# SandeepaInduwaraSamaranayake/SwinVox

Hardware: AMD Instinct MI355X
Metric: views/sec fwd+bwd SwinVox-T 224^2, 32^3 voxel, n_views=8 (higher is better)
Workload: dtype bf16; 1 GPU; SwinVox-T full pipeline (ResNet50[:layer3] || Swin multi-stage, cross-view attention, decoder, merger, refiner), fwd+2xBCE+bwd, train mode, B=64 samples x V=8 views of 224x224 per GPU; global_batch=64, n_views=8, images_per_gpu=512, parallelism=single GPU, launch=eager (one host launch per kernel, three streams)

## Files before the change

swinvox_amd/csrc/stencil.hip:

```cpp
#include "common.h"
#include <map>
#include <mutex>
#include <type_traits>

namespace sv {

constexpr int TZ = 4, TY = 8, TX = 8;
constexpr int HZ = TZ + 2, HY = TY + 2, HX = TX + 2;
constexpr int HPOS = HZ * HY * HX;
constexpr int NVOX = TZ * TY * TX;
typedef __attribute__((address_space(3))) bf16x4 lds_bf16x4_t;

__device__ __forceinline__ bf16x4 to_bf16x4(float4 v) {
  bf16x4 b;
  b[0] = (__bf16)v.x; b[1] = (__bf16)v.y; b[2] = (__bf16)v.z; b[3] = (__bf16)v.w;
  return b;
}
__device__ __forceinline__ bf16x4 to_bf16x4(bf16x4 v) { return v; }

__device__ __forceinline__ int xcd_first_tile() {
  const int n = gridDim.x, b = blockIdx.x;
  return (n & 7) == 0 ? (b & 7) * (n >> 3) + (b >> 3) : b;
}

struct TileId { int img, z0, y0, x0; };
template <int TZV = TZ>
__device__ __forceinline__ TileId tile_of(int t, int D, int H, int W) {
  const int tz = D / TZV, ty = H / TY, tx = W / TX;
  TileId r;
  r.x0 = (t % tx) * TX; t /= tx; r.y0 = (t % ty) * TY; t /= ty; r.z0 = (t % tz) * TZV; r.img = t / tz;
  return r;
}

template <int G, typename AT, int TZV = TZ, int NTHR = 256>
struct HaloRegs {
  static constexpr int HZV = TZV + 2, HPOSV = HZV * HY * HX;
  static constexpr int C = 16 * G, VPP = C / 4, N = (HPOSV * VPP + NTHR - 1) / NTHR;
  typedef typename std::conditional<G == 1, int, long long>::type OffT;
  typename V4<AT>::type r[N];
  OffT off[N];
  int face[N];
  int lds[N];
  __device__ __forceinline__ void init(int ldx, long long plane, int cin_load, int H, int W, int tid, int pitch = HX) {
#pragma unroll
    for (int k = 0; k < N; ++k) {
      const int i = tid + NTHR * k;
      const int h = i / VPP, v = i - h * VPP;
      const int hx = h % HX; const int t2 = h / HX; const int hy = t2 % HY; const int hz = t2 / HY;
      const int cv = v * 4, pl = plane ? cv / ldx : 0;
      face[k] = (hz == 0 ? 1 : 0) | (hz == HZV - 1 ? 2 : 0) | (hy == 0 ? 4 : 0) | (hy == HY - 1 ? 8 : 0) | (hx == 0 ? 16 : 0) | (hx == HX - 1 ? 32 : 0) |
                ((i < HPOSV * VPP && cv < cin_load) ? 0 : 64);
      off[k] = (OffT)pl * (OffT)plane + (OffT)(((hz * H + hy) * W + hx) * ldx + (cv - pl * ldx));
      lds[k] = ((hz * HY + hy) * pitch + hx) * C + cv;
    }
  }
  __device__ __forceinline__ void load(const AT* __restrict__ x, int ldx, const TileId& t, int D, int H, int W) {
    const int out = (t.z0 == 0 ? 1 : 0) | (t.z0 + TZV == D ? 2 : 0) | (t.y0 == 0 ? 4 : 0) | (t.y0 + TY == H ? 8 : 0) | (t.x0 == 0 ? 16 : 0) | (t.x0 + TX == W ? 32 : 0) | 64;
    const AT* corner = x + ((((long long)t.img * D + t.z0 - 1) * H + t.y0 - 1) * W + t.x0 - 1) * (long long)ldx;
#pragma unroll
    for (int k = 0; k < N; ++k) {
      typename V4<AT>::type q = V4<AT>::zero();
#ifndef SV_ST_PROBE_NOLOAD
      if ((face[k] & out) == 0) q = V4<AT>::load(corner + off[k]);
#endif
      r[k] = q;
    }
  }
  __device__ __forceinline__ void store(__bf16* Xs, int tid) const {
#pragma unroll
    for (int k = 0; k < N; ++k) {
      const int i = tid + NTHR * k;
      if (i < HPOSV * VPP) *reinterpret_cast<bf16x4*>(Xs + lds[k]) = to_bf16x4(r[k]);
    }
  }
};

template <typename AT>
struct StencilArgsT {
  const AT* x; int ldx; int cin_load;
  long long x_plane, out_plane;
  const __bf16* w;
  const float* bias; AT* out; int ldc; int col_off; int cout;
  const AT* residual; int ldr;
  double* stats;
  int I, D, H, W, ntiles;
};

template <int G> struct StencilPitch { static constexpr int HXP = G == 1 ? 16 : HX; };
template <int G> struct StencilBrick { static constexpr int TZV = 8, NTHR = TZV * 64; };
template <int G> struct StencilBrickF { static constexpr int TZV = 8, NTHR = TZV * 64; };
template <int G, int NT, typename AT, bool VEC>
__global__ __launch_bounds__(StencilBrickF<G>::NTHR, 2) void stencil3_fwd_kernel(const StencilArgsT<AT> p) {
  constexpr int C = 16 * G, KTOT = 27 * C, KPAD = (KTOT + 31) / 32 * 32, NSTEP = KPAD / 32, HXP = StencilPitch<G>::HXP;
  constexpr int TZV = StencilBrickF<G>::TZV, NTHR = StencilBrickF<G>::NTHR, NW = NTHR / 64;
  __shared__ __attribute__((aligned(16))) char xc[(TZV + 2) * HY * HXP * C * 2];
  __shared__ __attribute__((aligned(16))) __bf16 Ws[NT * 16 * KPAD];
  __shared__ float red[16 * 16 * 2];
  __bf16* Xs = reinterpret_cast<__bf16*>(xc);
  const int tid = threadIdx.x, lane = tid & 63, wave = tid >> 6;
  const int lr = lane & 15, lg = lane >> 4;

  for (int i = tid; i < NT * 16 * KPAD / 8; i += NTHR) {
    const int n = (i * 8) / KPAD, k = (i * 8) - n * KPAD;
    bf16x8 v = VecN<__bf16, 8>::zero();
    if (k < KTOT) v = *reinterpret_cast<const bf16x8*>(p.w + (size_t)n * KTOT + k);
    *reinterpret_cast<bf16x8*>(Ws + n * KPAD + k) = v;
  }
  const int cs4 = (p.cout + 3) & ~3;
  float bias4[NT][4], st1[4] = {0.f, 0.f, 0.f, 0.f}, st2[4] = {0.f, 0.f, 0.f, 0.f};
#pragma unroll
  for (int nt = 0; nt < NT; ++nt)
#pragma unroll
    for (int j = 0; j < 4; ++j) { const int n = nt * 16 + lg * 4 + j; bias4[nt][j] = (p.bias && n < p.cout) ? p.bias[n] : 0.f; }

  HaloRegs<G, AT, TZV, NTHR> hr;
  hr.init(p.ldx, p.x_plane, p.cin_load, p.H, p.W, tid, HXP);
  int tile = xcd_first_tile();
  TileId t = tile_of<TZV>(tile < p.ntiles ? tile : 0, p.D, p.H, p.W);
  if (tile < p.ntiles) { hr.load(p.x, p.ldx, t, p.D, p.H, p.W); hr.store(Xs, tid); }
  __syncthreads();
  const int yy = lr >> 3, xx = lr & 7;
  int toff[NSTEP];
#pragma unroll
  for (int s = 0; s < NSTEP; ++s) {
    const int kb = s * 32 + lg * 8;
    int tap = kb / C; const int c = kb - tap * C;
    if (tap > 26) tap = 26;
    const int dz = tap / 9, dy = (tap - dz * 9) / 3, dx = tap - dz * 9 - dy * 3;
    toff[s] = (((dz * HY + dy) * HXP + dx) * C + c) * 2;
  }
  const char* xrow = xc + ((wave * HY + yy) * HXP + xx) * C * 2;
  const char* wrow = reinterpret_cast<const char*>(Ws) + (lr * KPAD + lg * 8) * 2;
  const int n0 = lg * 4;
  bool colreal[NT][4];
#pragma unroll
  for (int nt = 0; nt < NT; ++nt)
#pragma unroll
    for (int j = 0; j < 4; ++j) colreal[nt][j] = nt * 16 + n0 + j < p.cout;
  for (; tile < p.ntiles; tile += gridDim.x) {
    const int next = tile + gridDim.x;
    TileId tn = t;
    if (next < p.ntiles) { tn = tile_of<TZV>(next, p.D, p.H, p.W); hr.load(p.x, p.ldx, tn, p.D, p.H, p.W); }

    f32x4 acc[4][NT];
#pragma unroll
    for (int mt = 0; mt < 4; ++mt)
#pragma unroll
      for (int nt = 0; nt < NT; ++nt) acc[mt][nt] = (f32x4){0.f, 0.f, 0.f, 0.f};
#ifndef SV_ST_PROBE_NOMMA
#pragma unroll
    for (int s = 0; s < NSTEP; ++s) {
      bf16x8 b[NT];
#pragma unroll
      for (int nt = 0; nt < NT; ++nt) b[nt] = *reinterpret_cast<const bf16x8*>(wrow + nt * 16 * KPAD * 2 + s * 64);
      const char* ap = xrow + toff[s];
#pragma unroll
      for (int mt = 0; mt < 4; ++mt) {
        const bf16x8 a = *reinterpret_cast<const bf16x8*>(ap + mt * (2 * HXP * C * 2));
#pragma unroll
        for (int nt = 0; nt < NT; ++nt) acc[mt][nt] = __builtin_amdgcn_mfma_f32_16x16x32_bf16(b[nt], a, acc[mt][nt], 0, 0, 0);
      }
    }
#endif
    const size_t pos0 = (((size_t)t.img * p.D + t.z0 + wave) * p.H + t.y0 + yy) * p.W + t.x0 + xx;
    if constexpr (VEC) {
#pragma unroll
      for (int nt = 0; nt < NT; ++nt) {
        const int nn = nt * 16 + n0;
        if (nn >= cs4) continue;
        AT* orow; const AT* rrow = nullptr;
        if (p.out_plane) { const int pl = nn / p.ldc; orow = p.out + (size_t)pl * p.out_plane + pos0 * p.ldc + (nn - pl * p.ldc); }
        else orow = p.out + pos0 * p.ldc + p.col_off + nn;
        if (p.residual) rrow = p.residual + pos0 * p.ldr + nn;
#pragma unroll
        for (int mt = 0; mt < 4; ++mt) {
          float v[4];
#pragma unroll
          for (int j = 0; j < 4; ++j) v[j] = colreal[nt][j] ? acc[mt][nt][j] + bias4[nt][j] : 0.f;
          if (NT == 1 && p.stats) {
#pragma unroll
            for (int j = 0; j < 4; ++j) { st1[j] += v[j]; st2[j] += v[j] * v[j]; }
          }
          if (p.residual) {
            const float4 rv = ld4f(rrow + (size_t)mt * 2 * p.W * p.ldr);
            v[0] += rv.x; v[1] += rv.y; v[2] += rv.z; v[3] += rv.w;
          }
#ifdef SV_ST_PROBE_NOSTORE
          if (v[0] == 1234.5f)
#endif
          st4f(orow + (size_t)mt * 2 * p.W * p.ldc, make_float4(v[0], v[1], v[2], v[3]));
        }
      }
    } else {
#pragma unroll
      for (int mt = 0; mt < 4; ++mt) {
        const size_t pos = pos0 + (size_t)mt * 2 * p.W;
#pragma unroll
        for (int nt = 0; nt < NT; ++nt) {
          const int nn = nt * 16 + n0;
#pragma unroll
          for (int j = 0; j < 4; ++j) {
            if (nn + j < p.cout) {
              float r = acc[mt][nt][j] + bias4[nt][j];
              if (NT == 1 && p.stats) { st1[j] += r; st2[j] += r * r; }
              if (p.residual) r += ldf(p.residual + pos * p.ldr + nn + j);
              stf(p.out + pos * p.ldc + p.col_off + nn + j, r);
            }
          }
        }
      }
    }
    t = tn;
    __syncthreads();
    if (next < p.ntiles) hr.store(Xs, tid);
    __syncthreads();
  }
  if (NT == 1 && p.stats) {
#pragma unroll
    for (int j = 0; j < 4; ++j) {
      { st1[j] += dpp_move<0xB1>(st1[j]); st1[j] += dpp_move<0x4E>(st1[j]); st1[j] += dpp_move<0x141>(st1[j]); st1[j] += dpp_move<0x140>(st1[j]);
        st2[j] += dpp_move<0xB1>(st2[j]); st2[j] += dpp_move<0x4E>(st2[j]); st2[j] += dpp_move<0x141>(st2[j]); st2[j] += dpp_move<0x140>(st2[j]); }
    }
    if (lr == 0) {
#pragma unroll
      for (int j = 0; j < 4; ++j) { red[(wave * 16 + lg * 4 + j) * 2] = st1[j]; red[(wave * 16 + lg * 4 + j) * 2 + 1] = st2[j]; }
    }
    __syncthreads();
    if (tid < 16 && tid < p.cout) {
      float a = 0.f, b = 0.f;
#pragma unroll
      for (int w = 0; w < NW; ++w) { a += red[(w * 16 + tid) * 2]; b += red[(w * 16 + tid) * 2 + 1]; }
      double* st = p.stats + (size_t)(blockIdx.x % SV_BN_SLOTS) * 2 * p.cout;
      atomicAdd(st + tid, (double)a);
      atomicAdd(st + p.cout + tid, (double)b);
    }
  }
}

template <typename AT>
struct StencilWArgsT {
  const AT* x; int ldx; int cin_load;
  long long x_plane;
  const AT* dy; int lddy; int cout_load;
  float* dw;
  float* ws;
  float* dbias;
  int cout, cin;
  int c_stride, c_valid;
  int I, D, H, W, ntiles;
};

constexpr int WG_SLOTS = 16;
__global__ __launch_bounds__(256) void stencil_wgrad_fold_kernel(const float* __restrict__ ws, float* __restrict__ dw, int n) {
  const int i = blockIdx.x * 256 + threadIdx.x;
  if (i >= n) return;
  float a = 0.f;
#pragma unroll
  for (int sl = 0; sl < WG_SLOTS; ++sl) a += ws[(size_t)sl * n + i];
  dw[i] += a;
}

template <int G, typename AT>
__global__ __launch_bounds__(StencilBrick<G>::NTHR, 2) void stencil3_wgrad_kernel(const StencilWArgsT<AT> p) {
  constexpr int C = 16 * G, TZV = StencilBrick<G>::TZV, NTHR = StencilBrick<G>::NTHR, NW = NTHR / 64, NTAPW = (27 + NW - 1) / NW;
  constexpr int HPOSV = (TZV + 2) * HY * HX, NVOXV = TZV * TY * TX;
  __shared__ __attribute__((aligned(16))) __bf16 Xs[HPOSV * C];
  __shared__ __attribute__((aligned(16))) __bf16 Ds[NVOXV * 16];
  __shared__ float bred[NTHR / 16 * 16];
  const int tid = threadIdx.x, lane = tid & 63, wave = tid >> 6;
  const int lr = lane & 15, lg = lane >> 4, q = lr >> 2, pp = lr & 3;
  const int ntap = (27 - wave + NW - 1) / NW;
  f32x4 acc[NTAPW][G];
#pragma unroll
  for (int i = 0; i < NTAPW; ++i)
#pragma unroll
    for (int gg = 0; gg < G; ++gg) acc[i][gg] = (f32x4){0.f, 0.f, 0.f, 0.f};
  float bsum = 0.f;

  HaloRegs<G, AT, TZV, NTHR> hr;
  hr.init(p.ldx, p.x_plane, p.cin_load, p.H, p.W, tid);
  typename V4<AT>::type dr[4];
  auto load_dy = [&](const TileId& t) {
#pragma unroll
    for (int k = 0; k < 4; ++k) {
      const int i = tid + NTHR * k;
      const int v = i >> 2, c4 = i & 3;
      const int xx = v % TX; const int t2 = v / TX; const int yy = t2 % TY; const int zz = t2 / TY;
      typename V4<AT>::type qv = V4<AT>::zero();
      if (c4 * 4 < p.cout_load)
        qv = V4<AT>::load(p.dy + ((((size_t)t.img * p.D + t.z0 + zz) * p.H + t.y0 + yy) * p.W + t.x0 + xx) * (size_t)p.lddy + c4 * 4);
      dr[k] = qv;
    }
  };
  auto store_dy = [&]() {
#pragma unroll
    for (int k = 0; k < 4; ++k) *reinterpret_cast<bf16x4*>(Ds + (tid + NTHR * k) * 4) = to_bf16x4(dr[k]);
  };

  int tile = xcd_first_tile();
  if (tile < p.ntiles) {
    const TileId t = tile_of<TZV>(tile, p.D, p.H, p.W);
    hr.load(p.x, p.ldx, t, p.D, p.H, p.W); load_dy(t);
    hr.store(Xs, tid); store_dy();
  }
  __syncthreads();
  for (; tile < p.ntiles; tile += gridDim.x) {
    const int next = tile + gridDim.x;
    if (next < p.ntiles) {
      const TileId t = tile_of<TZV>(next, p.D, p.H, p.W);
      hr.load(p.x, p.ldx, t, p.D, p.H, p.W); load_dy(t);
    }
    if (p.dbias) {
      const int c = tid & 15, vg = tid >> 4;
#pragma unroll
      for (int k = 0; k < 16; ++k) bsum += (float)Ds[(vg * 16 + k) * 16 + c];
    }
#pragma unroll 1
    for (int ch = 0; ch < 2 * TZV; ++ch) {
      const int z = ch >> 1, yb = (ch & 1) * 4 + lg;
      const __bf16* asrc = Ds + (((z * TY + yb) * TX) + q) * 16 + pp * 4;
      const bf16x4 alo = __builtin_amdgcn_ds_read_tr16_b64_v4bf16((lds_bf16x4_t*)(asrc));
      const bf16x4 ahi = __builtin_amdgcn_ds_read_tr16_b64_v4bf16((lds_bf16x4_t*)(asrc + 4 * 16));
      const bf16x8 a = __builtin_shufflevector(alo, ahi, 0, 1, 2, 3, 4, 5, 6, 7);
#pragma unroll
      for (int i = 0; i < NTAPW; ++i) {
        if (i < ntap) {
          const int tap = wave + NW * i;
          const int dz = tap / 9, dy = (tap - dz * 9) / 3, dx = tap - dz * 9 - dy * 3;
          const int hb = ((z + dz) * HY + yb + dy) * HX + dx + q;
#pragma unroll
          for (int gg = 0; gg < G; ++gg) {
            const __bf16* bsrc = Xs + hb * C + gg * 16 + pp * 4;
            const bf16x4 blo = __builtin_amdgcn_ds_read_tr16_b64_v4bf16((lds_bf16x4_t*)(bsrc));
            const bf16x4 bhi = __builtin_amdgcn_ds_read_tr16_b64_v4bf16((lds_bf16x4_t*)(bsrc + 4 * C));
            const bf16x8 b = __builtin_shufflevector(blo, bhi, 0, 1, 2, 3, 4, 5, 6, 7);
            acc[i][gg] = __builtin_amdgcn_mfma_f32_16x16x32_bf16(a, b, acc[i][gg], 0, 0, 0);
          }
        }
      }
    }
    __syncthreads();
    if (next < p.ntiles) { hr.store(Xs, tid); store_dy(); }
    __syncthreads();
  }
  if (p.dbias) {
    bred[tid] = bsum;
    __syncthreads();
    if (tid < 16 && tid < p.cout) {
      float a = 0.f;
#pragma unroll
      for (int g2 = 0; g2 < NTHR / 16; ++g2) a += bred[g2 * 16 + tid];
      atomicAdd(p.dbias + tid, a);
    }
  }
  float* dst = p.ws ? p.ws + (size_t)(blockIdx.x % WG_SLOTS) * p.cout * p.cin * 27 : p.dw;
#pragma unroll
  for (int i = 0; i < NTAPW; ++i) {
    if (i < ntap) {
      const int tap = wave + NW * i;
#pragma unroll
      for (int gg = 0; gg < G; ++gg) {
        const int cm = gg * 16 + lr;
        const int grp = cm / p.c_stride, within = cm - grp * p.c_stride;
        const int ci = grp * p.c_valid + within;
        if (within < p.c_valid && ci < p.cin) {
#pragma unroll
          for (int j = 0; j < 4; ++j) {
            const int co = lg * 4 + j;
            if (co < p.cout) atomicAdd(dst + ((size_t)co * p.cin + ci) * 27 + tap, acc[i][gg][j]);
          }
        }
      }
    }
  }
}

struct TConv4Args {
  const __bf16* x; const __bf16* w;
  const float* bias; __bf16* out; double* stats; int cout; int I, D, H, W, nbricks;
};
constexpr int T4_JZ = 4, T4_JY = 4, T4_JX = 8, T4_HZ = 6, T4_HY = 6, T4_HX = 10, T4_HPOS = T4_HZ * T4_HY * T4_HX;

__global__ __launch_bounds__(256, 2) void tconv4s2_fwd_kernel(const TConv4Args p) {
  __shared__ __attribute__((aligned(16))) __bf16 Xs[T4_HPOS * 32];
  __shared__ __attribute__((aligned(16))) __bf16 Ws[8 * 8 * 256];
  __shared__ __attribute__((aligned(16))) __bf16 Os[8 * 8 * 16 * 8];
  __shared__ float red[4][16];
  const int tid = threadIdx.x, lane = tid & 63, wave = tid >> 6;
  const int lr = lane & 15, lg = lane >> 4;
  for (int i = tid; i < 8 * 8 * 256 / 8; i += 256) {
    const int c8 = (i & 3) * 8, t = (i >> 2) & 7, co = (i >> 5) & 7, cls = i >> 8;
    const int az = cls >> 2, ay = (cls >> 1) & 1, ax = cls & 1, dz = t >> 2, dy = (t >> 1) & 1, dx = t & 1;
    const int kz = az ? 2 - 2 * dz : 3 - 2 * dz, ky = ay ? 2 - 2 * dy : 3 - 2 * dy, kx = ax ? 2 - 2 * dx : 3 - 2 * dx;
    bf16x8 v = VecN<__bf16, 8>::zero();
    if (co < p.cout) v = *reinterpret_cast<const bf16x8*>(p.w + ((size_t)co * 64 + (kz * 4 + ky) * 4 + kx) * 32 + c8);
    *reinterpret_cast<bf16x8*>(Ws + ((cls * 8 + co) * 256) + t * 32 + c8) = v;
  }
  float bias4[4];
#pragma unroll
  for (int j = 0; j < 4; ++j) bias4[j] = (p.bias && lg < 2 && lg * 4 + j < p.cout) ? p.bias[lg * 4 + j] : 0.f;
  double st1[8], st2[8];
#pragma unroll
  for (int c = 0; c < 8; ++c) { st1[c] = 0.0; st2[c] = 0.0; }
  const int bz = p.D / T4_JZ, by = p.H / T4_JY, bx = p.W / T4_JX;
  __syncthreads();
  for (int brick = blockIdx.x; brick < p.nbricks; brick += gridDim.x) {
    int t = brick;
    const int x0 = (t % bx) * T4_JX; t /= bx;
    const int y0 = (t % by) * T4_JY; t /= by;
    const int z0 = (t % bz) * T4_JZ; const int img = t / bz;
    for (int i = tid; i < T4_HPOS * 4; i += 256) {
      const int h = i >> 2, c8 = (i & 3) * 8;
      const int hx = h % T4_HX; const int t2 = h / T4_HX; const int hy = t2 % T4_HY; const int hz = t2 / T4_HY;
      const int z = z0 - 1 + hz, y = y0 - 1 + hy, xx = x0 - 1 + hx;
      bf16x8 v = VecN<__bf16, 8>::zero();
      if ((unsigned)z < (unsigned)p.D && (unsigned)y < (unsigned)p.H && (unsigned)xx < (unsigned)p.W)
        v = *reinterpret_cast<const bf16x8*>(p.x + ((((size_t)img * p.D + z) * p.H + y) * p.W + xx) * 32 + c8);
      *reinterpret_cast<bf16x8*>(Xs + h * 32 + c8) = v;
    }
    __syncthreads();
    const int yy = lr >> 3, xx = lr & 7;
#pragma unroll 1
    for (int ci = 0; ci < 2; ++ci) {
      const int cls = 2 * wave + ci, az = cls >> 2, ay = (cls >> 1) & 1, ax = cls & 1;
      bf16x8 b[8];
#pragma unroll
      for (int tt = 0; tt < 8; ++tt) {
        b[tt] = VecN<__bf16, 8>::zero();
        if (lr < 8) b[tt] = *reinterpret_cast<const bf16x8*>(Ws + (cls * 8 + lr) * 256 + tt * 32 + lg * 8);
      }
#pragma unroll 2
      for (int g = 0; g < 8; ++g) {
        const int jz = g >> 1, jy = (g & 1) * 2 + yy;
        const int base = ((jz + az) * T4_HY + (jy + ay)) * T4_HX + (xx + ax);
        f32x4 acc = (f32x4){0.f, 0.f, 0.f, 0.f};
#pragma unroll
        for (int tt = 0; tt < 8; ++tt) {
          const int off = ((tt >> 2) * T4_HY + ((tt >> 1) & 1)) * T4_HX + (tt & 1);
          const bf16x8 a = *reinterpret_cast<const bf16x8*>(Xs + (base + off) * 32 + lg * 8);
          acc = __builtin_amdgcn_mfma_f32_16x16x32_bf16(b[tt], a, acc, 0, 0, 0);
        }
        if (lg < 2) {
          bf16x4 o;
#pragma unroll
          for (int j = 0; j < 4; ++j) o[j] = (__bf16)(acc[j] + bias4[j]);
          const int oz = 2 * jz + az, oy = 2 * jy + ay, ox = 2 * xx + ax;
          *reinterpret_cast<bf16x4*>(Os + ((oz * 8 + oy) * 16 + ox) * 8 + lg * 4) = o;
        }
      }
    }
    __syncthreads();
#pragma unroll
    for (int k = 0; k < 4; ++k) {
      const int v = tid + 256 * k;
      const int ox = v & 15, oy = (v >> 4) & 7, oz = v >> 7;
      const bf16x8 o = *reinterpret_cast<const bf16x8*>(Os + v * 8);
      const size_t pos = (((size_t)img * (2 * p.D) + 2 * z0 + oz) * (2 * p.H) + 2 * y0 + oy) * (2 * p.W) + 2 * x0 + ox;
      *reinterpret_cast<bf16x8*>(p.out + pos * 8) = o;
      if (p.stats) {
#pragma unroll
        for (int c = 0; c < 8; ++c) { const double f = (double)(float)o[c]; st1[c] += f; st2[c] += f * f; }
      }
    }
    __syncthreads();
  }
  if (p.stats) {
#pragma unroll
    for (int c = 0; c < 8; ++c) {
      float a = (float)st1[c], b2 = (float)st2[c];
      a = wave_sum(a); b2 = wave_sum(b2);
      if (lane == 0) { red[wave][c] = a; red[wave][8 + c] = b2; }
    }
    __syncthreads();
    if (tid < 16 && (tid & 7) < p.cout) {
      const float v = red[0][tid] + red[1][tid] + red[2][tid] + red[3][tid];
      double* st = p.stats + (size_t)(blockIdx.x % SV_BN_SLOTS) * 2 * p.cout;
      atomicAdd(st + (tid >> 3) * p.cout + (tid & 7), (double)v);
    }
  }
}

}

using namespace sv;

static int resident_per_cu(const void* kernel, int threads = 256) {
  static std::mutex mu;
  static std::map<const void*, int> cache;
  std::lock_guard<std::mutex> lk(mu);
  auto it = cache.find(kernel);
  if (it != cache.end()) return it->second;
  int n = 0;
  if (hipOccupancyMaxActiveBlocksPerMultiprocessor(&n, kernel, threads, 0) != hipSuccess || n < 1) { (void)hipGetLastError(); n = 1; }
  cache[kernel] = n;
  return n;
}

static int stencil_check(int I, int D, int H, int W) {
  SV_REQUIRE(I > 0 && D % 8 == 0 && H % TY == 0 && W % TX == 0, "stencil3: grid %dx%dx%d must be a multiple of the 8x8x8 brick", D, H, W);
  return SV_OK;
}

#define SV_STENCIL_LAUNCH(GG, NTT, VV)                                                                                     \
  do {                                                                                                                    \
    constexpr int nthr = StencilBrickF<GG>::NTHR;                                                                         \
    const int nt_ = I * (D / StencilBrickF<GG>::TZV) * (H / TY) * (W / TX);                                               \
    a.ntiles = nt_;                                                                                                       \
    const int resident = 256 * resident_per_cu((const void*)stencil3_fwd_kernel<GG, NTT, AT, VV>, nthr);                  \
    hipLaunchKernelGGL((stencil3_fwd_kernel<GG, NTT, AT, VV>), dim3(nt_ < resident ? nt_ : resident), dim3(nthr), 0, s, a); \
  } while (0)

extern "C" int sv_stencil3_fwd(const void* x, int ldx, int cin_load, int groups, const void* w_bf16, int ntiles16,
                               const float* bias, void* out, int ldc, int col_off, int cout, const void* residual, int ldr,
                               double* stats, int I, int D, int H, int W, long long x_plane_stride, long long out_plane_stride,
                               int act_dtype, void* stream) {
  SV_REQUIRE(x && w_bf16 && out, "stencil3_fwd: null argument");
  SV_REQUIRE(x_plane_stride >= 0 && out_plane_stride >= 0 && x_plane_stride % 4 == 0 && out_plane_stride % 4 == 0, "stencil3_fwd: bad plane strides");
  SV_REQUIRE(!out_plane_stride || (col_off == 0 && !residual && ldc % 4 == 0 && cout % ldc == 0),
             "stencil3_fwd: planar output needs col_off == 0, no residual and whole planes of ldc (multiple of 4) columns");
  SV_REQUIRE_ACT(act_dtype);
  if (int rc = stencil_check(I, D, H, W)) return rc;
    SV_REQUIRE(cin_load % 4 == 0 && cin_load <= 16 * groups && ldx % 4 == 0 && (x_plane_stride ? cin_load % ldx == 0 : ldx >= cin_load),
             "stencil3_fwd: bad input channels (cin_load=%d ldx=%d groups=%d)", cin_load, ldx, groups);
  SV_REQUIRE(cout > 0 && cout <= 16 * ntiles16 && (out_plane_stride || ldc >= col_off + cout), "stencil3_fwd: bad output window");
  SV_REQUIRE(!stats || ntiles16 == 1, "stencil3_fwd: statistics need a single 16-column tile");
  const uintptr_t amask = act_dtype == SV_BF16 ? 7 : 15;
  SV_REQUIRE(((uintptr_t)x & amask) == 0 && ((uintptr_t)w_bf16 & 15) == 0, "stencil3_fwd: operands must be aligned to 4 elements");
  SV_REQUIRE((ldc & 3) != 0 || (((uintptr_t)out | (uintptr_t)residual) & amask) == 0,
             "stencil3_fwd: out/residual must be aligned to 4 elements when ldc is a multiple of 4");
  const int ntiles = I * (D / TZ) * (H / TY) * (W / TX);
  hipStream_t s = (hipStream_t)stream;
  if (!((groups == 1 && ntiles16 == 1) || (groups == 3 && ntiles16 == 1) || (groups == 1 && ntiles16 == 3))) {
    set_error("stencil3_fwd: unsupported (groups=%d, ntiles16=%d)", groups, ntiles16);
    return SV_ERR_INVALID;
  }
  SV_DISPATCH_ACT(act_dtype,
    const int cs4 = (cout + 3) & ~3;
    const bool vec = out_plane_stride != 0 || ((ldc & 3) == 0 && (col_off & 3) == 0 && col_off + cs4 <= ldc && (!residual || ((ldr & 3) == 0 && cs4 <= ldr)));
    StencilArgsT<AT> a{static_cast<const AT*>(x), ldx, cin_load, x_plane_stride, out_plane_stride, (const __bf16*)w_bf16, bias, static_cast<AT*>(out), ldc, col_off, cout,
                       static_cast<const AT*>(residual), ldr, stats, I, D, H, W, ntiles};
    if (groups == 1 && ntiles16 == 1) { if (vec) SV_STENCIL_LAUNCH(1, 1, true); else SV_STENCIL_LAUNCH(1, 1, false); }
    else if (groups == 3) { if (vec) SV_STENCIL_LAUNCH(3, 1, true); else SV_STENCIL_LAUNCH(3, 1, false); }
    else { if (vec) SV_STENCIL_LAUNCH(1, 3, true); else SV_STENCIL_LAUNCH(1, 3, false); });
  return check_launch("sv_stencil3_fwd");
}

extern "C" size_t sv_stencil3_wgrad_workspace_floats(int cout, int cin) { return (size_t)WG_SLOTS * cout * cin * 27; }

extern "C" int sv_stencil3_wgrad(const void* x, int ldx, int cin_load, int groups, const void* dy, int lddy, int cout_load,
                                 float* dw, float* dbias, float* workspace, int cout, int cin, int c_stride, int c_valid, int I, int D, int H,
                                 int W, long long x_plane_stride, int act_dtype, void* stream) {
  SV_REQUIRE(x && dy && dw, "stencil3_wgrad: null argument");
  SV_REQUIRE(x_plane_stride >= 0 && x_plane_stride % 4 == 0 && (!x_plane_stride || cin_load % ldx == 0), "stencil3_wgrad: bad plane stride");
  SV_REQUIRE_ACT(act_dtype);
  if (int rc = stencil_check(I, D, H, W)) return rc;
  SV_REQUIRE(cin_load % 4 == 0 && cin_load <= 16 * groups && ldx % 4 == 0 && cout_load % 4 == 0 && cout_load <= 16 && lddy % 4 == 0,
             "stencil3_wgrad: bad channel layout");
  SV_REQUIRE(cout > 0 && cout <= 16 && cin > 0 && c_stride > 0 && c_valid > 0, "stencil3_wgrad: bad channel counts");
  SV_REQUIRE((((uintptr_t)x | (uintptr_t)dy) & (act_dtype == SV_BF16 ? 7 : 15)) == 0, "stencil3_wgrad: operands must be aligned to 4 elements");
  SV_REQUIRE(groups == 1 || groups == 3, "stencil3_wgrad: unsupported groups=%d", groups);
    const int ntiles = I * (D / (groups == 3 ? StencilBrick<3>::TZV : StencilBrick<1>::TZV)) * (H / TY) * (W / TX);
  hipStream_t s = (hipStream_t)stream;
  SV_DISPATCH_ACT(act_dtype,
    const int per_cu = groups == 1 ? resident_per_cu((const void*)stencil3_wgrad_kernel<1, AT>, StencilBrick<1>::NTHR)
                                   : resident_per_cu((const void*)stencil3_wgrad_kernel<3, AT>, StencilBrick<3>::NTHR);
    const int resident = 256 * per_cu;
    const int blocks = ntiles < resident ? ntiles : resident;
    StencilWArgsT<AT> a{static_cast<const AT*>(x), ldx, cin_load, x_plane_stride, static_cast<const AT*>(dy), lddy, cout_load, dw, workspace, dbias, cout, cin, c_stride, c_valid,
                        I, D, H, W, ntiles};
    if (groups == 1) hipLaunchKernelGGL((stencil3_wgrad_kernel<1, AT>), dim3(blocks), dim3(StencilBrick<1>::NTHR), 0, s, a);
    else hipLaunchKernelGGL((stencil3_wgrad_kernel<3, AT>), dim3(blocks), dim3(StencilBrick<3>::NTHR), 0, s, a););
  if (workspace) hipLaunchKernelGGL(stencil_wgrad_fold_kernel, dim3(cdiv(cout * cin * 27, 256)), dim3(256), 0, s, workspace, dw, cout * cin * 27);
  return check_launch("sv_stencil3_wgrad");
}

extern "C" int sv_tconv4s2_fwd(const void* x, const void* w_packed, const float* bias, void* out, double* stats, int I, int D, int H, int W,
                               int cin, int cout, void* stream) {
  SV_REQUIRE(x && w_packed && out && I > 0, "tconv4s2_fwd: null argument");
  SV_REQUIRE(cin == 32 && cout > 0 && cout <= 8, "tconv4s2_fwd: built for 32 input and <= 8 output channels (got %d -> %d)", cin, cout);
  SV_REQUIRE(D % T4_JZ == 0 && H % T4_JY == 0 && W % T4_JX == 0, "tconv4s2_fwd: input grid %dx%dx%d must be a multiple of the 4x4x8 brick", D, H, W);
  SV_REQUIRE((((uintptr_t)x | (uintptr_t)w_packed | (uintptr_t)out) & 15) == 0, "tconv4s2_fwd: operands must be 16-byte aligned");
  TConv4Args a{static_cast<const __bf16*>(x), static_cast<const __bf16*>(w_packed), bias, static_cast<__bf16*>(out), stats, cout, I, D, H, W,
               I * (D / T4_JZ) * (H / T4_JY) * (W / T4_JX)};
  const int blocks = a.nbricks < 512 ? a.nbricks : 512;
  hipLaunchKernelGGL(tconv4s2_fwd_kernel, dim3(blocks), dim3(256), 0, (hipStream_t)stream, a);
  return check_launch("sv_tconv4s2_fwd");
}
```

Baseline: 4896 views/s.

## Add z-sweep wgrad kernel for 3x3x3 stencil reusing dy slices across taps

Adds a new weight-gradient kernel for the 3D stencil conv, enabled by default with an env opt-out. Each wave owns a pair of in-plane taps and sweeps the z slices of a brick, reusing each loaded dy and x fragment across the three dz taps via MFMA with transposed LDS reads. The halo loader is restructured into z-slice groups so fewer per-thread offsets are held in registers. The two y-halves combine their accumulators through LDS before the atomics. The trade-offs are more accumulator registers, a different occupancy setting and added code complexity.

```diff
diff --git a/swinvox_amd/csrc/stencil.hip b/swinvox_amd/csrc/stencil.hip
--- a/swinvox_amd/csrc/stencil.hip
+++ b/swinvox_amd/csrc/stencil.hip
@@ -72,6 +72,67 @@
       const int i = tid + NTHR * k;
       if (i < HPOSV * VPP) *reinterpret_cast<bf16x4*>(Xs + lds[k]) = to_bf16x4(r[k]);
     }
+  }
+};
+
+template <int G, typename AT, int TZV, int NTHR>
+struct HaloSliceRegs {
+  static constexpr int HZV = TZV + 2, C = 16 * G, VPP = C / 4;
+  static constexpr int ZG = G == 1 ? 5 : 2, NGRP = HZV / ZG, GV = ZG * HY * HX * VPP, NP = (GV + NTHR - 1) / NTHR, N = NGRP * NP;
+  static_assert(HZV % ZG == 0, "groups of whole z-slices");
+  static_assert(HZV * HY * 16 * C < (1 << 20), "LDS offsets (pitch <= 16 positions) take 20 bits");
+  typename V4<AT>::type r[N];
+  int off[NP], meta[NP];
+  long long plane_;
+  int gstep_, lstep_;
+  __device__ __forceinline__ void init(int ldx, long long plane, int cin_load, int H, int W, int tid, int pitch) {
+#pragma unroll
+    for (int j = 0; j < NP; ++j) {
+      const int i = tid + NTHR * j;
+      int h = i / VPP, v = i - h * VPP;
+      const int nvp = ldx / 4;
+      if (plane && VPP % nvp == 0) {
+        const int row = i / (HX * VPP), rem = i - row * (HX * VPP);
+        const int pq = rem / (HX * nvp), r2 = rem - pq * (HX * nvp), px = r2 / nvp;
+        h = row * HX + px; v = pq * nvp + (r2 - px * nvp);
+      }
+      const int hx = h % HX; const int t2 = h / HX; const int hy = t2 % HY; const int hz = t2 / HY;
+      const int cv = v * 4, pl = plane ? cv / ldx : 0;
+      const int fc = (hz == 0 ? 1 : 0) | (hz == ZG - 1 ? 2 : 0) | (hy == 0 ? 4 : 0) | (hy == HY - 1 ? 8 : 0) | (hx == 0 ? 16 : 0) | (hx == HX - 1 ? 32 : 0) |
+                     ((i < GV && cv < cin_load) ? 0 : 64);
+      const int lo = i < GV ? ((hz * HY + hy) * pitch + hx) * C + cv : 0;
+      meta[j] = lo | (fc << 20) | (pl << 27);
+      off[j] = ((hz * H + hy) * W + hx) * ldx + (cv - pl * ldx);
+    }
+    plane_ = plane; gstep_ = ZG * H * W * ldx; lstep_ = ZG * HY * pitch * C;
+  }
+  __device__ __forceinline__ void load(const AT* __restrict__ x, int ldx, const TileId& t, int D, int H, int W) {
+    const int zlo = t.z0 == 0 ? 1 : 0, zhi = t.z0 + TZV == D ? 2 : 0;
+    const int yx = (t.y0 == 0 ? 4 : 0) | (t.y0 + TY == H ? 8 : 0) | (t.x0 == 0 ? 16 : 0) | (t.x0 + TX == W ? 32 : 0) | 64;
+    const AT* corner = x + ((((long long)t.img * D + t.z0 - 1) * H + t.y0 - 1) * W + t.x0 - 1) * (long long)ldx;
+#pragma unroll
+    for (int g = 0; g < NGRP; ++g) {
+      const int out = (yx | (g == 0 ? zlo : 0) | (g == NGRP - 1 ? zhi : 0)) << 20;
+      const AT* cg = corner + (long long)g * gstep_;
+#pragma unroll
+      for (int j = 0; j < NP; ++j) {
+        typename V4<AT>::type q = V4<AT>::zero();
+#ifndef SV_ST_PROBE_NOLOAD
+        if ((meta[j] & out) == 0) {
+          if constexpr (G > 1) q = V4<AT>::load(cg + (long long)((meta[j] >> 27) & 15) * plane_ + off[j]);
+          else q = V4<AT>::load(cg + off[j]);
+        }
+#endif
+        r[g * NP + j] = q;
+      }
+    }
+  }
+  __device__ __forceinline__ void store(__bf16* Xs, int tid) const {
+#pragma unroll
+    for (int g = 0; g < NGRP; ++g)
+#pragma unroll
+      for (int j = 0; j < NP; ++j)
+        if ((j + 1) * NTHR <= GV || tid + NTHR * j < GV) *reinterpret_cast<bf16x4*>(Xs + g * lstep_ + (meta[j] & 0xfffff)) = to_bf16x4(r[g * NP + j]);
   }
 };
 
@@ -368,6 +429,184 @@
           for (int j = 0; j < 4; ++j) {
             const int co = lg * 4 + j;
             if (co < p.cout) atomicAdd(dst + ((size_t)co * p.cin + ci) * 27 + tap, acc[i][gg][j]);
+          }
+        }
+      }
+    }
+  }
+}
+
+#ifdef SV_ST_PROBE_WG_PITCH
+constexpr int SWEEP_HXP = SV_ST_PROBE_WG_PITCH;
+#else
+constexpr int SWEEP_HXP = 12;
+#endif
+#ifdef SV_ST_PROBE_WG_LA
+constexpr int SWEEP_LA = SV_ST_PROBE_WG_LA;
+#else
+constexpr int SWEEP_LA = 1;
+#endif
+#ifdef SV_ST_PROBE_WG_NOSWAP
+constexpr int SWEEP_DYSWAP = 0;
+#else
+constexpr int SWEEP_DYSWAP = 4;
+#endif
+template <int G, typename AT>
+__global__ __launch_bounds__(StencilBrick<G>::NTHR, G == 1 && sizeof(AT) == 2 ? 4 : 2) void stencil3_wgrad_sweep_kernel(const StencilWArgsT<AT> p) {
+  constexpr int C = 16 * G, TZV = StencilBrick<G>::TZV, NTHR = StencilBrick<G>::NTHR, HXP = SWEEP_HXP;
+  constexpr int XELEMS = (TZV + 2) * HY * HXP * C, NVOXV = TZV * TY * TX, LA = SWEEP_LA;
+  static_assert(NTHR == 512 && NTHR * 4 == NVOXV * 4, "8 waves: 2 y-halves x 4 pair slots; dy staging = 4 vectors per thread");
+  static_assert(4 * 9 * G * 64 * 4 * sizeof(float) <= XELEMS * sizeof(__bf16), "the half-1 accumulators are handed over through the x image");
+  __shared__ __attribute__((aligned(16))) __bf16 Xs[XELEMS];
+  __shared__ __attribute__((aligned(16))) __bf16 Ds[NVOXV * 16];
+  __shared__ float bred[2 * 64];
+  const int tid = threadIdx.x, lane = tid & 63, wave = __builtin_amdgcn_readfirstlane(tid >> 6);
+  const int lr = lane & 15, lg = lane >> 4, q = lr >> 2, pp = lr & 3;
+  const int half = wave & 1, slot = wave >> 1;
+  const int p0 = slot ? 1 + 2 * slot : 0;
+  const bool three = slot == 0, sums_bias = p.dbias != nullptr && slot == 1;
+  f32x4 acc[3][3][G];
+#pragma unroll
+  for (int pi = 0; pi < 3; ++pi)
+#pragma unroll
+    for (int dz = 0; dz < 3; ++dz)
+#pragma unroll
+      for (int gg = 0; gg < G; ++gg) acc[pi][dz][gg] = (f32x4){0.f, 0.f, 0.f, 0.f};
+  float bsum = 0.f;
+
+  HaloSliceRegs<G, AT, TZV, NTHR> hr;
+  hr.init(p.ldx, p.x_plane, p.cin_load, p.H, p.W, tid, HXP);
+  typename V4<AT>::type dr[4];
+  const int dv0 = tid >> 2, dc4 = (tid & 3) * 4;
+  const int dyoff = (((dv0 / (TY * TX)) * p.H + (dv0 / TX) % TY) * p.W + dv0 % TX) * p.lddy + dc4;
+  const int dystep = 2 * p.H * p.W * p.lddy;
+  auto load_dy = [&](const TileId& t) {
+    const AT* d0 = p.dy + ((((size_t)t.img * p.D + t.z0) * p.H + t.y0) * p.W + t.x0) * (size_t)p.lddy + dyoff;
+#pragma unroll
+    for (int k = 0; k < 4; ++k) {
+      typename V4<AT>::type qv = V4<AT>::zero();
+      if (dc4 < p.cout_load) qv = V4<AT>::load(d0 + (size_t)k * dystep);
+      dr[k] = qv;
+    }
+  };
+  auto store_dy = [&]() {
+#pragma unroll
+    for (int k = 0; k < 4; ++k) {
+      const int i = tid + NTHR * k;
+      const int v = i >> 2, vs = v ^ (((v >> 3) & 1) * SWEEP_DYSWAP);
+      *reinterpret_cast<bf16x4*>(Ds + vs * 16 + (i & 3) * 4) = to_bf16x4(dr[k]);
+    }
+  };
+  const int yb = 4 * half + lg;
+  const __bf16* xsrc[3];
+#pragma unroll
+  for (int pi = 0; pi < 3; ++pi) {
+    const int pr = (pi < 2 || three) ? p0 + pi : p0;
+    const int dy = pr / 3, dx = pr - dy * 3;
+    xsrc[pi] = Xs + ((yb + dy) * HXP + dx + q) * C + pp * 4;
+  }
+  const __bf16* alo_src = Ds + (yb * TX + q + ((yb & 1) ? SWEEP_DYSWAP : 0)) * 16 + pp * 4;
+  const __bf16* ahi_src = Ds + (yb * TX + q + 4 - ((yb & 1) ? SWEEP_DYSWAP : 0)) * 16 + pp * 4;
+
+  auto read_dy = [&](int z) {
+    const bf16x4 alo = __builtin_amdgcn_ds_read_tr16_b64_v4bf16((lds_bf16x4_t*)(alo_src + z * TY * TX * 16));
+    const bf16x4 ahi = __builtin_amdgcn_ds_read_tr16_b64_v4bf16((lds_bf16x4_t*)(ahi_src + z * TY * TX * 16));
+    return (bf16x8)__builtin_shufflevector(alo, ahi, 0, 1, 2, 3, 4, 5, 6, 7);
+  };
+  auto read_x = [&](int s, int pi, int gg) {
+    const __bf16* bsrc = xsrc[pi] + s * HY * HXP * C + gg * 16;
+    const bf16x4 blo = __builtin_amdgcn_ds_read_tr16_b64_v4bf16((lds_bf16x4_t*)(bsrc));
+    const bf16x4 bhi = __builtin_amdgcn_ds_read_tr16_b64_v4bf16((lds_bf16x4_t*)(bsrc + 4 * C));
+    return (bf16x8)__builtin_shufflevector(blo, bhi, 0, 1, 2, 3, 4, 5, 6, 7);
+  };
+  auto sweep = [&](auto PI0, auto NPI) {
+    constexpr int pi0 = decltype(PI0)::value, npi = decltype(NPI)::value, NSTEP = (TZV + 2) * npi * G;
+    bf16x8 a[4];
+    bf16x8 b[LA + 1];
+    a[0] = read_dy(0);
+#pragma unroll
+    for (int n = 0; n < LA; ++n) b[n] = read_x(n / (npi * G), pi0 + (n / G) % npi, n % G);
+#pragma unroll
+    for (int n = 0; n < NSTEP; ++n) {
+      const int s = n / (npi * G), pi = pi0 + (n / G) % npi, gg = n % G;
+      if (n % (npi * G) == 0 && s + 1 < TZV) a[(s + 1) % 4] = read_dy(s + 1);
+      if (n + LA < NSTEP) b[(n + LA) % (LA + 1)] = read_x((n + LA) / (npi * G), pi0 + ((n + LA) / G) % npi, (n + LA) % G);
+      __builtin_amdgcn_sched_barrier(0);
+#pragma unroll
+      for (int dz = 0; dz < 3; ++dz)
+        if (s - dz >= 0 && s - dz < TZV) acc[pi][dz][gg] = __builtin_amdgcn_mfma_f32_16x16x32_bf16(a[(s - dz) % 4], b[n % (LA + 1)], acc[pi][dz][gg], 0, 0, 0);
+      __builtin_amdgcn_sched_barrier(0);
+    }
+  };
+
+  int tile = xcd_first_tile();
+  if (tile < p.ntiles) {
+    const TileId t = tile_of<TZV>(tile, p.D, p.H, p.W);
+    hr.load(p.x, p.ldx, t, p.D, p.H, p.W); load_dy(t);
+    hr.store(Xs, tid); store_dy();
+  }
+  __syncthreads();
+  for (; tile < p.ntiles; tile += gridDim.x) {
+    const int next = tile + gridDim.x;
+    if (next < p.ntiles) {
+      const TileId t = tile_of<TZV>(next, p.D, p.H, p.W);
+      hr.load(p.x, p.ldx, t, p.D, p.H, p.W); load_dy(t);
+    }
+#ifndef SV_ST_PROBE_NOMMA
+    sweep(std::integral_constant<int, 0>(), std::integral_constant<int, 2>());
+    if (three) sweep(std::integral_constant<int, 2>(), std::integral_constant<int, 1>());
+    if (sums_bias) {
+#pragma unroll
+      for (int z = 0; z < TZV; ++z) {
+        const bf16x8 a = read_dy(z);
+        float t8 = 0.f;
+#pragma unroll
+        for (int j = 0; j < 8; ++j) t8 += (float)a[j];
+        bsum += t8;
+      }
+    }
+#endif
+    __syncthreads();
+    if (next < p.ntiles) { hr.store(Xs, tid); store_dy(); }
+    __syncthreads();
+  }
+  f32x4* hand = reinterpret_cast<f32x4*>(Xs) + (size_t)slot * 9 * G * 64 + lane;
+  if (half == 1) {
+#pragma unroll
+    for (int pi = 0; pi < 3; ++pi)
+#pragma unroll
+      for (int dz = 0; dz < 3; ++dz)
+#pragma unroll
+        for (int gg = 0; gg < G; ++gg) hand[((pi * 3 + dz) * G + gg) * 64] = acc[pi][dz][gg];
+  }
+  if (sums_bias) bred[half * 64 + lane] = bsum;
+  __syncthreads();
+  if (p.dbias && tid < 16 && tid < p.cout) {
+    float s8 = 0.f;
+#pragma unroll
+    for (int g2 = 0; g2 < 8; ++g2) s8 += bred[g2 * 16 + tid];
+    atomicAdd(p.dbias + tid, s8);
+  }
+  if (half == 1) return;
+  float* dst = p.ws ? p.ws + (size_t)(blockIdx.x % WG_SLOTS) * p.cout * p.cin * 27 : p.dw;
+#pragma unroll
+  for (int pi = 0; pi < 3; ++pi) {
+    if (pi < 2 || three) {
+#pragma unroll
+      for (int dz = 0; dz < 3; ++dz) {
+        const int tap = dz * 9 + p0 + pi;
+#pragma unroll
+        for (int gg = 0; gg < G; ++gg) {
+          const f32x4 o = hand[((pi * 3 + dz) * G + gg) * 64];
+          const int cm = gg * 16 + lr;
+          const int grp = cm / p.c_stride, within = cm - grp * p.c_stride;
+          const int ci = grp * p.c_valid + within;
+          if (within < p.c_valid && ci < p.cin) {
+#pragma unroll
+            for (int j = 0; j < 4; ++j) {
+              const int co = lg * 4 + j;
+              if (co < p.cout) atomicAdd(dst + ((size_t)co * p.cin + ci) * 27 + tap, acc[pi][dz][gg][j] + o[j]);
+            }
           }
         }
       }
@@ -561,14 +800,19 @@
   SV_REQUIRE(groups == 1 || groups == 3, "stencil3_wgrad: unsupported groups=%d", groups);
     const int ntiles = I * (D / (groups == 3 ? StencilBrick<3>::TZV : StencilBrick<1>::TZV)) * (H / TY) * (W / TX);
   hipStream_t s = (hipStream_t)stream;
+  const char* sweep_env = getenv("SV_STENCIL_WGRAD_SWEEP");
+  const bool sweep = sweep_env ? atoi(sweep_env) != 0 : true;
   SV_DISPATCH_ACT(act_dtype,
-    const int per_cu = groups == 1 ? resident_per_cu((const void*)stencil3_wgrad_kernel<1, AT>, StencilBrick<1>::NTHR)
-                                   : resident_per_cu((const void*)stencil3_wgrad_kernel<3, AT>, StencilBrick<3>::NTHR);
+    const void* k1 = sweep ? (const void*)stencil3_wgrad_sweep_kernel<1, AT> : (const void*)stencil3_wgrad_kernel<1, AT>;
+    const void* k3 = sweep ? (const void*)stencil3_wgrad_sweep_kernel<3, AT> : (const void*)stencil3_wgrad_kernel<3, AT>;
+    const int per_cu = groups == 1 ? resident_per_cu(k1, StencilBrick<1>::NTHR) : resident_per_cu(k3, StencilBrick<3>::NTHR);
     const int resident = 256 * per_cu;
     const int blocks = ntiles < resident ? ntiles : resident;
     StencilWArgsT<AT> a{static_cast<const AT*>(x), ldx, cin_load, x_plane_stride, static_cast<const AT*>(dy), lddy, cout_load, dw, workspace, dbias, cout, cin, c_stride, c_valid,
                         I, D, H, W, ntiles};
-    if (groups == 1) hipLaunchKernelGGL((stencil3_wgrad_kernel<1, AT>), dim3(blocks), dim3(StencilBrick<1>::NTHR), 0, s, a);
+    if (groups == 1 && sweep) hipLaunchKernelGGL((stencil3_wgrad_sweep_kernel<1, AT>), dim3(blocks), dim3(StencilBrick<1>::NTHR), 0, s, a);
+    else if (groups == 1) hipLaunchKernelGGL((stencil3_wgrad_kernel<1, AT>), dim3(blocks), dim3(StencilBrick<1>::NTHR), 0, s, a);
+    else if (sweep) hipLaunchKernelGGL((stencil3_wgrad_sweep_kernel<3, AT>), dim3(blocks), dim3(StencilBrick<3>::NTHR), 0, s, a);
     else hipLaunchKernelGGL((stencil3_wgrad_kernel<3, AT>), dim3(blocks), dim3(StencilBrick<3>::NTHR), 0, s, a););
   if (workspace) hipLaunchKernelGGL(stencil_wgrad_fold_kernel, dim3(cdiv(cout * cin * 27, 256)), dim3(256), 0, s, workspace, dw, cout * cin * 27);
   return check_launch("sv_stencil3_wgrad");
```

Measured after the change: 4964 views/s, median of 6. +1.4%, better.
